# jontio/JAERO

Hardware: NVIDIA H100
Metric: IQ Msamples/s (10.5k OQPSK demod + Viterbi) (higher is better)
Workload: dtype f64

## Files before the change

### jaero_b200/csrc/cfe.cu

```cuda
#include "demod_device.cuh"
#include "fft_device.cuh"
#include <cooperative_groups.h>
#include <cstring>
#include <cstdio>
#include <cstdlib>

namespace jb {

static const int TILE = 16;
static const int MAXN = 128;
static const int CFE_THREADS = 256;

template <bool INV, int R>
__device__ __forceinline__ void stockham_pass(double2 (*s)[MAXN + 1], int n, int Ns, const double2 *__restrict__ tw, int tw_stride)
{
    stockham_pass<INV, R, TILE, MAXN + 1, CFE_THREADS>(s, n, Ns, tw, tw_stride);
}

template <bool INV>
__device__ __forceinline__ void tile_fft(double2 (*s)[MAXN + 1], int n, const double2 *__restrict__ tw, int tw_stride)
{
    stockham_pass<INV, 8>(s, n, 1, tw, tw_stride);
    if (n == 128) { stockham_pass<INV, 4>(s, n, 8, tw, tw_stride); stockham_pass<INV, 4>(s, n, 32, tw, tw_stride); }
    else if (n == 64) stockham_pass<INV, 8>(s, n, 8, tw, tw_stride);
    else stockham_pass<INV, 4>(s, n, 8, tw, tw_stride);
}

template <bool FUSED_INV_SQUARE>
__global__ void __launch_bounds__(CFE_THREADS)
cfe_col_kernel(CfePlan pl, const double2 *__restrict__ src, double2 *__restrict__ dst, size_t src_pitch, int rot, int ring_len, int ch0)
{
    __shared__ double2 s[TILE][MAXN + 1];
    const int ch = blockIdx.y;
    const int c0 = blockIdx.x * TILE;
    const int n1 = pl.n1, n2 = pl.n2, N = pl.nfft;
    const double2 *in = src + (size_t)(ch0 + ch) * src_pitch;
    double2 *out = dst + (size_t)ch * N;
    for (int e = threadIdx.x; e < n1 * TILE; e += CFE_THREADS) {
        const int r = e / TILE, cc = e - r * TILE;
        int n = n2 * r + c0 + cc;
        if (!FUSED_INV_SQUARE) { n += rot; if (n >= ring_len) n -= ring_len; }
        s[cc][r] = in[n];
    }
    __syncthreads();
    if (FUSED_INV_SQUARE) {
        tile_fft<true>(s, n1, pl.tw, N / n1);
        for (int e = threadIdx.x; e < n1 * TILE; e += CFE_THREADS) {
            const int cc = e / n1, r = e - cc * n1;
            const double2 x = s[cc][r];
            s[cc][r] = make_double2(x.x * x.x - x.y * x.y, x.x * x.y + x.y * x.x);
        }
        __syncthreads();
    }
    tile_fft<false>(s, n1, pl.tw, N / n1);
    for (int e = threadIdx.x; e < n1 * TILE; e += CFE_THREADS) {
        const int k1 = e / TILE, cc = e - k1 * TILE;
        const int c = c0 + cc;
        const double2 w = pl.tw[(c * k1) & (N - 1)];
        const double2 x = s[cc][k1];
        out[(size_t)k1 * n2 + c] = make_double2(x.x * w.x - x.y * w.y, x.x * w.y + x.y * w.x);
    }
}

__global__ void __launch_bounds__(CFE_THREADS)
cfe_row_mask_kernel(CfePlan pl, const double2 *__restrict__ src, double2 *__restrict__ dst)
{
    __shared__ double2 s[TILE][MAXN + 1];
    const int ch = blockIdx.y;
    const int r0 = blockIdx.x * TILE;
    const int n1 = pl.n1, n2 = pl.n2, N = pl.nfft;
    const double2 *in = src + (size_t)ch * N;
    double2 *out = dst + (size_t)ch * N;
    for (int e = threadIdx.x; e < n2 * TILE; e += CFE_THREADS) {
        const int rr = e / n2, c = e - rr * n2;
        s[rr][c] = in[(size_t)(r0 + rr) * n2 + c];
    }
    __syncthreads();
    tile_fft<false>(s, n2, pl.tw, N / n2);
    for (int e = threadIdx.x; e < n2 * TILE; e += CFE_THREADS) {
        const int rr = e / n2, k2 = e - rr * n2;
        const int k = (r0 + rr) + n1 * k2;
        double2 x = s[rr][k2];
        if (!pl.is8400) { if (k >= pl.startbin && k <= pl.stopbin) x = make_double2(0.0, 0.0); }
        else { const double w = pl.window[k]; x = make_double2(x.x * w, x.y * w); }
        s[rr][k2] = x;
    }
    __syncthreads();
    tile_fft<true>(s, n2, pl.tw, N / n2);
    for (int e = threadIdx.x; e < n2 * TILE; e += CFE_THREADS) {
        const int rr = e / n2, c = e - rr * n2;
        const int k1 = r0 + rr;
        double2 w = pl.tw[(c * k1) & (N - 1)];
        w.y = -w.y;
        const double2 x = s[rr][c];
        out[(size_t)k1 * n2 + c] = make_double2(x.x * w.x - x.y * w.y, x.x * w.y + x.y * w.x);
    }
}

__global__ void __launch_bounds__(CFE_THREADS)
cfe_row_logmag_kernel(CfePlan pl, DemodParams p, const double2 *__restrict__ src, int ch0)
{
    __shared__ double2 s[TILE][MAXN + 1];
    const int ch = blockIdx.y;
    const int r0 = blockIdx.x * TILE;
    const int n1 = pl.n1, n2 = pl.n2, N = pl.nfft;
    const double2 *in = src + (size_t)ch * N;
    double *y = pl.y + (size_t)(ch0 + ch) * N;
    const bool bigchange = p.I[(size_t)I_ZERO_BB * p.cpad + ch0 + ch] != 0;
    for (int e = threadIdx.x; e < n2 * TILE; e += CFE_THREADS) {
        const int rr = e / n2, c = e - rr * n2;
        s[rr][c] = in[(size_t)(r0 + rr) * n2 + c];
    }
    __syncthreads();
    tile_fft<false>(s, n2, pl.tw, N / n2);
    for (int e = threadIdx.x; e < n2 * TILE; e += CFE_THREADS) {
        const int k2 = e / TILE, rr = e - k2 * TILE;
        const int k1 = r0 + rr;
        const int k2s = (k2 + (n2 >> 1)) & (n2 - 1);
        const int i = k1 + n1 * k2s;
        const double2 x = s[rr][k2];
        const double mag = hypot(x.x, x.y);
        const double yo = bigchange ? 20.0 : y[i];
        y[i] = yo * 0.9 + 0.1 * 10 * log10(fmax(mag, 1.0));
    }
}

__global__ void __launch_bounds__(128)
cfe_search_kernel(CfePlan pl, DemodParams p)
{
    const int lane = threadIdx.x & 31;
    const int ch = blockIdx.x * (blockDim.x >> 5) + (threadIdx.x >> 5);
    if (ch >= p.n_channels) return;
    const double *y = pl.y + (size_t)ch * pl.nfft;
    const int N = pl.nfft, epb = pl.expectedpeakbin;
    double best = 0.0; int besti = 0x7fffffff;
    int i0 = pl.lo;
    if (pl.lo - epb - 1 >= 0 && pl.hi + epb + 1 < N) {
        for (; i0 + 128 <= pl.hi; i0 += 128) {
            double a[4][3], c[4][3];
#pragma unroll
            for (int u = 0; u < 4; u++) {
                const int i = i0 + lane + 32 * u;
#pragma unroll
                for (int j = -1; j <= 1; j++) { a[u][j + 1] = y[i - epb - j]; c[u][j + 1] = y[i + epb + j]; }
            }
#pragma unroll
            for (int u = 0; u < 4; u++) {
                double val = 0;
#pragma unroll
                for (int j = 0; j < 3; j++) val += (a[u][j] + c[u][j]);
                if (val > best) { best = val; besti = i0 + lane + 32 * u; }
            }
        }
    }
    for (int i = i0 + lane; i < pl.hi; i += 32) {
        if ((i < 0) || (i >= N)) continue;
        double val = 0;
        for (int j = -1; j <= 1; j++) {
            if (((i - epb - j) < 0) || ((i + epb + j) >= N)) continue;
            val += (y[i - epb - j] + y[i + epb + j]);
        }
        if (val > best) { best = val; besti = i; }
    }
    for (int off = 16; off > 0; off >>= 1) {
        const double ob = __shfl_xor_sync(0xffffffffu, best, off);
        const int oi = __shfl_xor_sync(0xffffffffu, besti, off);
        if (ob > best || (ob == best && oi < besti)) { best = ob; besti = oi; }
    }
    if (lane == 0) {
        const int zmaxloc = (best > 0.0) ? besti : N / 2;
        const double est = -((double)(zmaxloc - N / 2)) * pl.hzperbin * 0.5;
        p.D[(size_t)D_CFE_EST * p.cpad + ch] = est;
        int &emptying = p.I[(size_t)I_EMPTYING * p.cpad + ch];
        if (emptying <= 0) p.cfe_est_out[ch] = est;
        else { emptying--; p.cfe_est_out[ch] = 0.0; }
        p.I[(size_t)I_ZERO_BB * p.cpad + ch] = 0;
    }
}

namespace cgx = cooperative_groups;

static const int CC_CL = 8, CC_T = 256, CC_SEQ = 16, CC_RS = 143;
static const int CC_BUF = CC_SEQ * CC_RS * 16;
static const int CC_TW2 = 128, CC_TW3 = 152;
static const int CC_SM_TOTAL = 2 * CC_BUF + (128 + 24 + 32) * 16;

__device__ __forceinline__ int cc_ph(int e) { return e + (e >> 3); }

__device__ __forceinline__ double log10_ge1(double x)
{
    const double Lg1 = 6.666666666666735130e-01, Lg2 = 3.999999999940941908e-01, Lg3 = 2.857142874366239149e-01, Lg4 = 2.222219843214978396e-01,
                 Lg5 = 1.818357216161805012e-01, Lg6 = 1.531383769920937332e-01, Lg7 = 1.479819860511658591e-01;
    const double ivln10 = 4.34294481903251816668e-01, log10_2hi = 3.01029995663611771306e-01, log10_2lo = 3.69423907715893078616e-13;
    int hi = __double2hiint(x);
    const int lo = __double2loint(x);
    int k = (hi >> 20) - 1023;
    hi &= 0x000fffff;
    const int i = (hi + 0x95f64) & 0x100000;
    hi |= (i ^ 0x3ff00000);
    k += (i >> 20);
    const double f = __hiloint2double(hi, lo) - 1.0;
    const double s = div_fast(f, 2.0 + f);
    const double z = s * s, w = z * z;
    const double t1 = w * (Lg2 + w * (Lg4 + w * Lg6));
    const double t2 = z * (Lg1 + w * (Lg3 + w * (Lg5 + w * Lg7)));
    const double hfsq = 0.5 * f * f;
    const double lg = f - (hfsq - s * (hfsq + (t2 + t1)));
    const double dk = (double)k;
    return (dk * log10_2lo + ivln10 * lg) + dk * log10_2hi;
}

template <bool INV, bool FIRST, class Store>
__device__ __forceinline__ void cc_fft(double2 *__restrict__ buf, const double2 *__restrict__ tws, Store last)
{
    const int w = threadIdx.x >> 5, l = threadIdx.x & 31;
    if (FIRST) {
        double2 *row = buf + (w + ((l & 16) >> 1)) * CC_RS;
        const int j = l & 15;
        double2 v[8];
#pragma unroll
        for (int t = 0; t < 8; t++) v[t] = row[cc_ph(j + 16 * t)];
        __syncwarp();
        dft8<INV>(v);
#pragma unroll
        for (int t = 0; t < 8; t++) row[cc_ph(8 * j + t)] = v[t];
        __syncwarp();
    }
    double2 *r0 = buf + w * CC_RS, *r1 = buf + (w + 8) * CC_RS;
    auto radix4 = [&](double2 &v0, double2 &v1, double2 &v2, double2 &v3, double2 w1, double2 w2, double2 w3) {
        if (INV) { w1.y = -w1.y; w2.y = -w2.y; w3.y = -w3.y; }
        v1 = c_mul(v1, w1); v2 = c_mul(v2, w2); v3 = c_mul(v3, w3);
        dft4<INV>(v0, v1, v2, v3);
    };
    {
        double2 a0 = r0[cc_ph(l)], a1 = r0[cc_ph(l + 32)], a2 = r0[cc_ph(l + 64)], a3 = r0[cc_ph(l + 96)];
        double2 b0 = r1[cc_ph(l)], b1 = r1[cc_ph(l + 32)], b2 = r1[cc_ph(l + 64)], b3 = r1[cc_ph(l + 96)];
        __syncwarp();
        const int k = l & 7, ob = (l >> 3) * 32 + k;
        const double2 w1 = tws[CC_TW2 + k], w2 = tws[CC_TW2 + 8 + k], w3 = tws[CC_TW2 + 16 + k];
        radix4(a0, a1, a2, a3, w1, w2, w3); radix4(b0, b1, b2, b3, w1, w2, w3);
        r0[cc_ph(ob)] = a0; r0[cc_ph(ob + 8)] = a1; r0[cc_ph(ob + 16)] = a2; r0[cc_ph(ob + 24)] = a3;
        r1[cc_ph(ob)] = b0; r1[cc_ph(ob + 8)] = b1; r1[cc_ph(ob + 16)] = b2; r1[cc_ph(ob + 24)] = b3;
        __syncwarp();
    }
    {
        double2 a0 = r0[cc_ph(l)], a1 = r0[cc_ph(l + 32)], a2 = r0[cc_ph(l + 64)], a3 = r0[cc_ph(l + 96)];
        double2 b0 = r1[cc_ph(l)], b1 = r1[cc_ph(l + 32)], b2 = r1[cc_ph(l + 64)], b3 = r1[cc_ph(l + 96)];
        __syncwarp();
        const double2 w1 = tws[l], w2 = tws[CC_TW3 + l], w3 = tws[3 * l];
        radix4(a0, a1, a2, a3, w1, w2, w3); radix4(b0, b1, b2, b3, w1, w2, w3);
        last(w, l, a0); last(w, l + 32, a1); last(w, l + 64, a2); last(w, l + 96, a3);
        last(w + 8, l, b0); last(w + 8, l + 32, b1); last(w + 8, l + 64, b2); last(w + 8, l + 96, b3);
        __syncwarp();
    }
}

__global__ void __launch_bounds__(CC_T, 2)
cfe_cluster_kernel(CfePlan pl, DemodParams p, int oldest)
{
    extern __shared__ __align__(128) unsigned char cc_smem[];
    double2 *bufA = reinterpret_cast<double2 *>(cc_smem);
    double2 *bufB = reinterpret_cast<double2 *>(cc_smem + CC_BUF);
    double2 *tws = reinterpret_cast<double2 *>(cc_smem + 2 * CC_BUF);
    cgx::cluster_group cluster = cgx::this_cluster();
    const int q = (int)cluster.block_rank();
    const int n_clusters = gridDim.x / CC_CL, cid = blockIdx.x / CC_CL;
    const int N = 16384, ring_len = p.bb_len;
    const double2 *__restrict__ twN = pl.tw;
    if (threadIdx.x < 128) tws[threadIdx.x] = twN[threadIdx.x * (N / 128)];
    else if (threadIdx.x < 128 + 24) { const int e = threadIdx.x - 128, m = e >> 3, k = e & 7; tws[CC_TW2 + e] = twN[(4 * (m + 1) * k) * (N / 128)]; }
    else if (threadIdx.x < 128 + 24 + 32) { const int l = threadIdx.x - 152; tws[CC_TW3 + l] = twN[(2 * l) * (N / 128)]; }
    __syncthreads();
    const double2 *rA[CC_CL], *rB[CC_CL];
#pragma unroll
    for (int s = 0; s < CC_CL; s++) { rA[s] = cluster.map_shared_rank(bufA, s); rB[s] = cluster.map_shared_rank(bufB, s); }
    bool arrived = false;
    cluster.sync();
    for (int ch = cid; ch < p.n_channels; ch += n_clusters) {
        double2 colv[8];
        {
            const double2 *ring = p.bb + (size_t)ch * ring_len;
            const int cc = threadIdx.x & 15, r0i = threadIdx.x >> 4;
#pragma unroll
            for (int i = 0; i < 8; i++) {
                int n = oldest + 128 * (r0i + 16 * i) + 16 * q + cc;
                if (n >= ring_len) n -= ring_len;
                if (n >= ring_len) n -= ring_len;
                colv[i] = ring[n];
            }
        }
        dft8<false>(colv);
        if (arrived) { cluster.barrier_wait(); arrived = false; }
        {
            const int cc = threadIdx.x & 15, r0i = threadIdx.x >> 4;
#pragma unroll
            for (int i = 0; i < 8; i++) bufA[cc * CC_RS + cc_ph(8 * r0i + i)] = colv[i];
        }
        __syncthreads();
        cc_fft<false, false>(bufA, tws, [&](int f, int e, double2 v) { bufA[f * CC_RS + cc_ph(e)] = v; });
        double2 tw8[8];
        {
            const int kk = threadIdx.x & 15, cc = threadIdx.x >> 4;
#pragma unroll
            for (int s = 0; s < 8; s++) tw8[s] = __ldg(&twN[((16 * s + cc) * (16 * q + kk)) & (N - 1)]);
        }
        cluster.sync();
        {
            const int kk = threadIdx.x & 15, cc = threadIdx.x >> 4;
            double2 x[8];
#pragma unroll
            for (int s = 0; s < 8; s++) x[s] = c_mul(rA[s][cc * CC_RS + cc_ph(16 * q + kk)], tw8[s]);
            dft8<false>(x);
#pragma unroll
            for (int s = 0; s < 8; s++) bufB[kk * CC_RS + cc_ph(8 * cc + s)] = x[s];
        }
        __syncthreads();
        cc_fft<false, false>(bufB, tws, [&](int f, int e, double2 v) {
            const int k = (16 * q + f) + 128 * e;
            if (!pl.is8400) { if (k >= pl.startbin && k <= pl.stopbin) v = make_double2(0.0, 0.0); }
            else { const double w = pl.window[k]; v = make_double2(v.x * w, v.y * w); }
            bufB[f * CC_RS + cc_ph(e)] = v;
        });
        cc_fft<true, true>(bufB, tws, [&](int f, int e, double2 v) { bufB[f * CC_RS + cc_ph(e)] = v; });
        {
            const int cc = threadIdx.x & 15, kk = threadIdx.x >> 4;
#pragma unroll
            for (int s = 0; s < 8; s++) tw8[s] = __ldg(&twN[((16 * q + cc) * (16 * s + kk)) & (N - 1)]);
        }
        cluster.sync();
        {
            const int cc = threadIdx.x & 15, kk = threadIdx.x >> 4;
            double2 x[8];
#pragma unroll
            for (int s = 0; s < 8; s++) {
                double2 w = tw8[s]; w.y = -w.y;
                x[s] = c_mul(rB[s][kk * CC_RS + cc_ph(16 * q + cc)], w);
            }
            dft8<true>(x);
#pragma unroll
            for (int s = 0; s < 8; s++) bufA[cc * CC_RS + cc_ph(8 * kk + s)] = x[s];
        }
        __syncthreads();
        cc_fft<true, false>(bufA, tws, [&](int f, int e, double2 v) {
            bufA[f * CC_RS + cc_ph(e)] = make_double2(v.x * v.x - v.y * v.y, v.x * v.y + v.y * v.x);
        });
        cc_fft<false, true>(bufA, tws, [&](int f, int e, double2 v) { bufA[f * CC_RS + cc_ph(e)] = v; });
        {
            const int kk = threadIdx.x & 15, cc = threadIdx.x >> 4;
#pragma unroll
            for (int s = 0; s < 8; s++) tw8[s] = __ldg(&twN[((16 * s + cc) * (16 * q + kk)) & (N - 1)]);
        }
        cluster.sync();
        {
            const int kk = threadIdx.x & 15, cc = threadIdx.x >> 4;
            double2 x[8];
#pragma unroll
            for (int s = 0; s < 8; s++) x[s] = c_mul(rA[s][cc * CC_RS + cc_ph(16 * q + kk)], tw8[s]);
            dft8<false>(x);
#pragma unroll
            for (int s = 0; s < 8; s++) bufB[kk * CC_RS + cc_ph(8 * cc + s)] = x[s];
        }
        cluster.barrier_arrive();
        arrived = true;
        __syncthreads();
        {
            double *y = pl.y + (size_t)ch * N;
            const bool bigchange = p.I[(size_t)I_ZERO_BB * p.cpad + ch] != 0;
            const int kk = threadIdx.x & 15, k2b = threadIdx.x >> 4;
            const int need_lo = pl.lo - pl.expectedpeakbin - 1, need_hi = pl.hi + pl.expectedpeakbin + 1;
            double yo[8];
#pragma unroll
            for (int i = 0; i < 8; i++) {
                const int i_sh = (16 * q + kk) + 128 * ((k2b + 16 * i + 64) & 127);
                yo[i] = (bigchange || i_sh < need_lo || i_sh > need_hi) ? 20.0 : y[i_sh];
            }
            cc_fft<false, false>(bufB, tws, [&](int f, int e, double2 v) { bufB[f * CC_RS + cc_ph(e)] = v; });
            __syncthreads();
#pragma unroll
            for (int i = 0; i < 8; i++) {
                const int k2 = k2b + 16 * i;
                const int i_sh = (16 * q + kk) + 128 * ((k2 + 64) & 127);
                if (i_sh < need_lo || i_sh > need_hi) continue;
                const double2 x = bufB[kk * CC_RS + cc_ph(k2)];
                y[i_sh] = yo[i] * 0.9 + 0.1 * 5 * log10_ge1(fmax(x.x * x.x + x.y * x.y, 1.0));
            }
        }
        __syncthreads();
    }
    if (arrived) cluster.barrier_wait();
    cluster.sync();
}

int cfe_cluster_run(const CfePlan &pl, const DemodParams &p, int oldest, int n_clusters, cudaStream_t s, long long *launches)
{
    cudaLaunchConfig_t cfg;
    memset(&cfg, 0, sizeof cfg);
    cfg.gridDim = dim3((unsigned)(n_clusters * CC_CL)); cfg.blockDim = dim3(CC_T); cfg.dynamicSmemBytes = CC_SM_TOTAL; cfg.stream = s;
    cudaLaunchAttribute at; at.id = cudaLaunchAttributeClusterDimension; at.val.clusterDim.x = CC_CL; at.val.clusterDim.y = 1; at.val.clusterDim.z = 1;
    cfg.attrs = &at; cfg.numAttrs = 1;
    JB_CUDA(cudaLaunchKernelEx(&cfg, cfe_cluster_kernel, pl, p, oldest));
    cfe_search_kernel<<<(p.n_channels + 3) / 4, 128, 0, s>>>(pl, p);
    JB_CUDA(cudaGetLastError());
    *launches += 2;
    return 0;
}
int cfe_cluster_capacity()
{
    if (cudaFuncSetAttribute(cfe_cluster_kernel, cudaFuncAttributeMaxDynamicSharedMemorySize, CC_SM_TOTAL) != cudaSuccess) { cudaGetLastError(); return 0; }
    cudaLaunchConfig_t cfg;
    memset(&cfg, 0, sizeof cfg);
    cfg.gridDim = dim3(CC_CL * 64); cfg.blockDim = dim3(CC_T); cfg.dynamicSmemBytes = CC_SM_TOTAL;
    cudaLaunchAttribute at; at.id = cudaLaunchAttributeClusterDimension; at.val.clusterDim.x = CC_CL; at.val.clusterDim.y = 1; at.val.clusterDim.z = 1;
    cfg.attrs = &at; cfg.numAttrs = 1;
    int n = 0;
    if (cudaOccupancyMaxActiveClusters(&n, cfe_cluster_kernel, &cfg) != cudaSuccess) { cudaGetLastError(); return 0; }
    if (getenv("JAERO_DEBUG")) fprintf(stderr, "[jaero_b200] estimator clusters co-resident: %d x %d CTAs\n", n, CC_CL);
    return n;
}

__global__ void cfe_mark_kernel(int *flag, int value) { __threadfence(); atomicExch(flag, value); }
int cfe_mark_launch(int *flag, int value, cudaStream_t s)
{
    cfe_mark_kernel<<<1, 1, 0, s>>>(flag, value);
    JB_CUDA(cudaGetLastError());
    return 0;
}

int cfe_run(const CfePlan &pl, const DemodParams &p, int oldest, cudaStream_t s, long long *launches)
{
    const int C = p.n_channels;
    for (int ch0 = 0; ch0 < C; ch0 += pl.group) {
        const int g = (C - ch0 < pl.group) ? C - ch0 : pl.group;
        dim3 gc(pl.n2 / TILE, g), gr(pl.n1 / TILE, g);
        cfe_col_kernel<false><<<gc, CFE_THREADS, 0, s>>>(pl, p.bb, pl.work_a, (size_t)p.bb_len, oldest, p.bb_len, ch0);
        cfe_row_mask_kernel<<<gr, CFE_THREADS, 0, s>>>(pl, pl.work_a, pl.work_b);
        cfe_col_kernel<true><<<gc, CFE_THREADS, 0, s>>>(pl, pl.work_b, pl.work_a, (size_t)pl.nfft, 0, pl.nfft, 0);
        cfe_row_logmag_kernel<<<gr, CFE_THREADS, 0, s>>>(pl, p, pl.work_a, ch0);
        *launches += 4;
    }
    cfe_search_kernel<<<(C + 3) / 4, 128, 0, s>>>(pl, p);
    *launches += 1;
    JB_CUDA(cudaGetLastError());
    return 0;
}

}
```

Baseline: 2278.

## Halve CFE cluster block size and fuse 128-point FFT passes in registers

Drops the cluster FFT kernel to 128 threads per block. Each thread now keeps 16 elements of a row in registers and runs the two radix-4 passes, and the radix-8 pass of the next transform, without a shared-memory round trip between them. The window/mask and squaring steps are applied in registers, and remote DSMEM pointers are mapped per access instead of cached in arrays. This trades fewer shared-memory passes and syncs for higher register pressure and half the threads per block, which may reduce occupancy and latency hiding.

Measured after the change: 2427 (median of 6 runs). 1.07x the previous value.

```diff
diff --git a/jaero_b200/csrc/cfe.cu b/jaero_b200/csrc/cfe.cu
--- a/jaero_b200/csrc/cfe.cu
+++ b/jaero_b200/csrc/cfe.cu
@@ -180,7 +180,7 @@
 
 namespace cgx = cooperative_groups;
 
-static const int CC_CL = 8, CC_T = 256, CC_SEQ = 16, CC_RS = 143;
+static const int CC_CL = 8, CC_T = 128, CC_SEQ = 16, CC_RS = 143;
 static const int CC_BUF = CC_SEQ * CC_RS * 16;
 static const int CC_TW2 = 128, CC_TW3 = 152;
 static const int CC_SM_TOTAL = 2 * CC_BUF + (128 + 24 + 32) * 16;
@@ -210,49 +210,57 @@
     return (dk * log10_2lo + ivln10 * lg) + dk * log10_2hi;
 }
 
-template <bool INV, bool FIRST, class Store>
-__device__ __forceinline__ void cc_fft(double2 *__restrict__ buf, const double2 *__restrict__ tws, Store last)
-{
-    const int w = threadIdx.x >> 5, l = threadIdx.x & 31;
-    if (FIRST) {
-        double2 *row = buf + (w + ((l & 16) >> 1)) * CC_RS;
-        const int j = l & 15;
-        double2 v[8];
-#pragma unroll
-        for (int t = 0; t < 8; t++) v[t] = row[cc_ph(j + 16 * t)];
-        __syncwarp();
-        dft8<INV>(v);
-#pragma unroll
-        for (int t = 0; t < 8; t++) row[cc_ph(8 * j + t)] = v[t];
-        __syncwarp();
-    }
-    double2 *r0 = buf + w * CC_RS, *r1 = buf + (w + 8) * CC_RS;
-    auto radix4 = [&](double2 &v0, double2 &v1, double2 &v2, double2 &v3, double2 w1, double2 w2, double2 w3) {
+__device__ __forceinline__ void cc_load16(const double2 *row, int k, double2 (&x)[16])
+{
+#pragma unroll
+    for (int p = 0; p < 16; p++) x[p] = row[cc_ph(k + 8 * p)];
+}
+
+__device__ __forceinline__ void cc_store16(double2 *row, int k, const double2 (&x)[16])
+{
+#pragma unroll
+    for (int p = 0; p < 16; p++) row[cc_ph(k + 8 * p)] = x[p];
+}
+
+template <bool INV>
+__device__ __forceinline__ void cc_pass23(double2 (&x)[16], int k, const double2 *__restrict__ tws)
+{
+    auto radix4 = [](double2 &v0, double2 &v1, double2 &v2, double2 &v3, double2 w1, double2 w2, double2 w3) {
         if (INV) { w1.y = -w1.y; w2.y = -w2.y; w3.y = -w3.y; }
         v1 = c_mul(v1, w1); v2 = c_mul(v2, w2); v3 = c_mul(v3, w3);
         dft4<INV>(v0, v1, v2, v3);
     };
+    double2 y[16];
     {
-        double2 a0 = r0[cc_ph(l)], a1 = r0[cc_ph(l + 32)], a2 = r0[cc_ph(l + 64)], a3 = r0[cc_ph(l + 96)];
-        double2 b0 = r1[cc_ph(l)], b1 = r1[cc_ph(l + 32)], b2 = r1[cc_ph(l + 64)], b3 = r1[cc_ph(l + 96)];
-        __syncwarp();
-        const int k = l & 7, ob = (l >> 3) * 32 + k;
         const double2 w1 = tws[CC_TW2 + k], w2 = tws[CC_TW2 + 8 + k], w3 = tws[CC_TW2 + 16 + k];
-        radix4(a0, a1, a2, a3, w1, w2, w3); radix4(b0, b1, b2, b3, w1, w2, w3);
-        r0[cc_ph(ob)] = a0; r0[cc_ph(ob + 8)] = a1; r0[cc_ph(ob + 16)] = a2; r0[cc_ph(ob + 24)] = a3;
-        r1[cc_ph(ob)] = b0; r1[cc_ph(ob + 8)] = b1; r1[cc_ph(ob + 16)] = b2; r1[cc_ph(ob + 24)] = b3;
-        __syncwarp();
-    }
-    {
-        double2 a0 = r0[cc_ph(l)], a1 = r0[cc_ph(l + 32)], a2 = r0[cc_ph(l + 64)], a3 = r0[cc_ph(l + 96)];
-        double2 b0 = r1[cc_ph(l)], b1 = r1[cc_ph(l + 32)], b2 = r1[cc_ph(l + 64)], b3 = r1[cc_ph(l + 96)];
-        __syncwarp();
-        const double2 w1 = tws[l], w2 = tws[CC_TW3 + l], w3 = tws[3 * l];
-        radix4(a0, a1, a2, a3, w1, w2, w3); radix4(b0, b1, b2, b3, w1, w2, w3);
-        last(w, l, a0); last(w, l + 32, a1); last(w, l + 64, a2); last(w, l + 96, a3);
-        last(w + 8, l, b0); last(w + 8, l + 32, b1); last(w + 8, l + 64, b2); last(w + 8, l + 96, b3);
-        __syncwarp();
-    }
+#pragma unroll
+        for (int m = 0; m < 4; m++) {
+            double2 v0 = x[m], v1 = x[m + 4], v2 = x[m + 8], v3 = x[m + 12];
+            radix4(v0, v1, v2, v3, w1, w2, w3);
+            y[4 * m] = v0; y[4 * m + 1] = v1; y[4 * m + 2] = v2; y[4 * m + 3] = v3;
+        }
+    }
+#pragma unroll
+    for (int u = 0; u < 4; u++) {
+        const int l = k + 8 * u;
+        double2 v0 = y[u], v1 = y[u + 4], v2 = y[u + 8], v3 = y[u + 12];
+        radix4(v0, v1, v2, v3, tws[l], tws[CC_TW3 + l], tws[3 * l]);
+        x[u] = v0; x[u + 4] = v1; x[u + 8] = v2; x[u + 12] = v3;
+    }
+}
+
+template <bool INV>
+__device__ __forceinline__ void cc_pass1_store(const double2 (&x)[16], double2 *row, int k)
+{
+    double2 a[8], b[8];
+#pragma unroll
+    for (int t = 0; t < 8; t++) { a[t] = x[2 * t]; b[t] = x[2 * t + 1]; }
+    dft8<INV>(a);
+    dft8<INV>(b);
+    __syncwarp();
+#pragma unroll
+    for (int t = 0; t < 8; t++) { row[cc_ph(8 * k + t)] = a[t]; row[cc_ph(8 * k + 64 + t)] = b[t]; }
+    __syncwarp();
 }
 
 __global__ void __launch_bounds__(CC_T, 2)
@@ -267,98 +275,137 @@
     const int n_clusters = gridDim.x / CC_CL, cid = blockIdx.x / CC_CL;
     const int N = 16384, ring_len = p.bb_len;
     const double2 *__restrict__ twN = pl.tw;
-    if (threadIdx.x < 128) tws[threadIdx.x] = twN[threadIdx.x * (N / 128)];
-    else if (threadIdx.x < 128 + 24) { const int e = threadIdx.x - 128, m = e >> 3, k = e & 7; tws[CC_TW2 + e] = twN[(4 * (m + 1) * k) * (N / 128)]; }
-    else if (threadIdx.x < 128 + 24 + 32) { const int l = threadIdx.x - 152; tws[CC_TW3 + l] = twN[(2 * l) * (N / 128)]; }
+    for (int t = threadIdx.x; t < 128 + 24 + 32; t += CC_T) {
+        if (t < 128) tws[t] = twN[t * (N / 128)];
+        else if (t < 128 + 24) { const int e = t - 128, m = e >> 3, k = e & 7; tws[CC_TW2 + e] = twN[(4 * (m + 1) * k) * (N / 128)]; }
+        else { const int l = t - 152; tws[CC_TW3 + l] = twN[(2 * l) * (N / 128)]; }
+    }
     __syncthreads();
-    const double2 *rA[CC_CL], *rB[CC_CL];
-#pragma unroll
-    for (int s = 0; s < CC_CL; s++) { rA[s] = cluster.map_shared_rank(bufA, s); rB[s] = cluster.map_shared_rank(bufB, s); }
     bool arrived = false;
     cluster.sync();
+    const int f = threadIdx.x >> 3, k = threadIdx.x & 7;
+    double2 *const rowA = bufA + f * CC_RS, *const rowB = bufB + f * CC_RS;
     for (int ch = cid; ch < p.n_channels; ch += n_clusters) {
-        double2 colv[8];
+        double2 x[16];
+        double2 colv[2][8];
         {
             const double2 *ring = p.bb + (size_t)ch * ring_len;
             const int cc = threadIdx.x & 15, r0i = threadIdx.x >> 4;
 #pragma unroll
-            for (int i = 0; i < 8; i++) {
-                int n = oldest + 128 * (r0i + 16 * i) + 16 * q + cc;
-                if (n >= ring_len) n -= ring_len;
-                if (n >= ring_len) n -= ring_len;
-                colv[i] = ring[n];
-            }
-        }
-        dft8<false>(colv);
+            for (int h = 0; h < 2; h++)
+#pragma unroll
+                for (int i = 0; i < 8; i++) {
+                    int n = oldest + 128 * (r0i + 8 * h + 16 * i) + 16 * q + cc;
+                    if (n >= ring_len) n -= ring_len;
+                    if (n >= ring_len) n -= ring_len;
+                    colv[h][i] = ring[n];
+                }
+        }
+        dft8<false>(colv[0]);
+        dft8<false>(colv[1]);
         if (arrived) { cluster.barrier_wait(); arrived = false; }
         {
             const int cc = threadIdx.x & 15, r0i = threadIdx.x >> 4;
 #pragma unroll
-            for (int i = 0; i < 8; i++) bufA[cc * CC_RS + cc_ph(8 * r0i + i)] = colv[i];
-        }
-        __syncthreads();
-        cc_fft<false, false>(bufA, tws, [&](int f, int e, double2 v) { bufA[f * CC_RS + cc_ph(e)] = v; });
-        double2 tw8[8];
+            for (int h = 0; h < 2; h++)
+#pragma unroll
+                for (int i = 0; i < 8; i++) bufA[cc * CC_RS + cc_ph(8 * (r0i + 8 * h) + i)] = colv[h][i];
+        }
+        __syncthreads();
+        cc_load16(rowA, k, x);
+        cc_pass23<false>(x, k, tws);
+        cc_store16(rowA, k, x);
+        double2 tw8[2][8];
         {
             const int kk = threadIdx.x & 15, cc = threadIdx.x >> 4;
 #pragma unroll
-            for (int s = 0; s < 8; s++) tw8[s] = __ldg(&twN[((16 * s + cc) * (16 * q + kk)) & (N - 1)]);
+            for (int h = 0; h < 2; h++)
+#pragma unroll
+                for (int s = 0; s < 8; s++) tw8[h][s] = __ldg(&twN[((16 * s + cc + 8 * h) * (16 * q + kk)) & (N - 1)]);
         }
         cluster.sync();
         {
+            const int kk = threadIdx.x & 15;
+#pragma unroll
+            for (int h = 0; h < 2; h++) {
+                const int cc = (threadIdx.x >> 4) + 8 * h;
+                double2 v[8];
+#pragma unroll
+                for (int s = 0; s < 8; s++) v[s] = c_mul(cluster.map_shared_rank(bufA, s)[cc * CC_RS + cc_ph(16 * q + kk)], tw8[h][s]);
+                dft8<false>(v);
+#pragma unroll
+                for (int s = 0; s < 8; s++) bufB[kk * CC_RS + cc_ph(8 * cc + s)] = v[s];
+            }
+        }
+        __syncthreads();
+        cc_load16(rowB, k, x);
+        cc_pass23<false>(x, k, tws);
+#pragma unroll
+        for (int e = 0; e < 16; e++) {
+            const int bin = (16 * q + f) + 128 * (k + 8 * e);
+            if (!pl.is8400) { if (bin >= pl.startbin && bin <= pl.stopbin) x[e] = make_double2(0.0, 0.0); }
+            else {
+                const double w = pl.window[bin];
+                x[e] = make_double2(__dmul_rn(x[e].x, w), __dmul_rn(x[e].y, w));
+            }
+        }
+        cc_pass1_store<true>(x, rowB, k);
+        cc_load16(rowB, k, x);
+        cc_pass23<true>(x, k, tws);
+        cc_store16(rowB, k, x);
+        {
+            const int cc = threadIdx.x & 15, kk = threadIdx.x >> 4;
+#pragma unroll
+            for (int h = 0; h < 2; h++)
+#pragma unroll
+                for (int s = 0; s < 8; s++) tw8[h][s] = __ldg(&twN[((16 * q + cc) * (16 * s + kk + 8 * h)) & (N - 1)]);
+        }
+        cluster.sync();
+        {
+            const int cc = threadIdx.x & 15;
+#pragma unroll
+            for (int h = 0; h < 2; h++) {
+                const int kk = (threadIdx.x >> 4) + 8 * h;
+                double2 v[8];
+#pragma unroll
+                for (int s = 0; s < 8; s++) {
+                    double2 w = tw8[h][s]; w.y = -w.y;
+                    v[s] = c_mul(cluster.map_shared_rank(bufB, s)[kk * CC_RS + cc_ph(16 * q + cc)], w);
+                }
+                dft8<true>(v);
+#pragma unroll
+                for (int s = 0; s < 8; s++) bufA[cc * CC_RS + cc_ph(8 * kk + s)] = v[s];
+            }
+        }
+        __syncthreads();
+        cc_load16(rowA, k, x);
+        cc_pass23<true>(x, k, tws);
+#pragma unroll
+        for (int e = 0; e < 16; e++) x[e] = make_double2(x[e].x * x[e].x - x[e].y * x[e].y, x[e].x * x[e].y + x[e].y * x[e].x);
+        cc_pass1_store<false>(x, rowA, k);
+        cc_load16(rowA, k, x);
+        cc_pass23<false>(x, k, tws);
+        cc_store16(rowA, k, x);
+        {
             const int kk = threadIdx.x & 15, cc = threadIdx.x >> 4;
-            double2 x[8];
-#pragma unroll
-            for (int s = 0; s < 8; s++) x[s] = c_mul(rA[s][cc * CC_RS + cc_ph(16 * q + kk)], tw8[s]);
-            dft8<false>(x);
-#pragma unroll
-            for (int s = 0; s < 8; s++) bufB[kk * CC_RS + cc_ph(8 * cc + s)] = x[s];
-        }
-        __syncthreads();
-        cc_fft<false, false>(bufB, tws, [&](int f, int e, double2 v) {
-            const int k = (16 * q + f) + 128 * e;
-            if (!pl.is8400) { if (k >= pl.startbin && k <= pl.stopbin) v = make_double2(0.0, 0.0); }
-            else { const double w = pl.window[k]; v = make_double2(v.x * w, v.y * w); }
-            bufB[f * CC_RS + cc_ph(e)] = v;
-        });
-        cc_fft<true, true>(bufB, tws, [&](int f, int e, double2 v) { bufB[f * CC_RS + cc_ph(e)] = v; });
-        {
-            const int cc = threadIdx.x & 15, kk = threadIdx.x >> 4;
-#pragma unroll
-            for (int s = 0; s < 8; s++) tw8[s] = __ldg(&twN[((16 * q + cc) * (16 * s + kk)) & (N - 1)]);
+#pragma unroll
+            for (int h = 0; h < 2; h++)
+#pragma unroll
+                for (int s = 0; s < 8; s++) tw8[h][s] = __ldg(&twN[((16 * s + cc + 8 * h) * (16 * q + kk)) & (N - 1)]);
         }
         cluster.sync();
         {
-            const int cc = threadIdx.x & 15, kk = threadIdx.x >> 4;
-            double2 x[8];
-#pragma unroll
-            for (int s = 0; s < 8; s++) {
-                double2 w = tw8[s]; w.y = -w.y;
-                x[s] = c_mul(rB[s][kk * CC_RS + cc_ph(16 * q + cc)], w);
-            }
-            dft8<true>(x);
-#pragma unroll
-            for (int s = 0; s < 8; s++) bufA[cc * CC_RS + cc_ph(8 * kk + s)] = x[s];
-        }
-        __syncthreads();
-        cc_fft<true, false>(bufA, tws, [&](int f, int e, double2 v) {
-            bufA[f * CC_RS + cc_ph(e)] = make_double2(v.x * v.x - v.y * v.y, v.x * v.y + v.y * v.x);
-        });
-        cc_fft<false, true>(bufA, tws, [&](int f, int e, double2 v) { bufA[f * CC_RS + cc_ph(e)] = v; });
-        {
-            const int kk = threadIdx.x & 15, cc = threadIdx.x >> 4;
-#pragma unroll
-            for (int s = 0; s < 8; s++) tw8[s] = __ldg(&twN[((16 * s + cc) * (16 * q + kk)) & (N - 1)]);
-        }
-        cluster.sync();
-        {
-            const int kk = threadIdx.x & 15, cc = threadIdx.x >> 4;
-            double2 x[8];
-#pragma unroll
-            for (int s = 0; s < 8; s++) x[s] = c_mul(rA[s][cc * CC_RS + cc_ph(16 * q + kk)], tw8[s]);
-            dft8<false>(x);
-#pragma unroll
-            for (int s = 0; s < 8; s++) bufB[kk * CC_RS + cc_ph(8 * cc + s)] = x[s];
+            const int kk = threadIdx.x & 15;
+#pragma unroll
+            for (int h = 0; h < 2; h++) {
+                const int cc = (threadIdx.x >> 4) + 8 * h;
+                double2 v[8];
+#pragma unroll
+                for (int s = 0; s < 8; s++) v[s] = c_mul(cluster.map_shared_rank(bufA, s)[cc * CC_RS + cc_ph(16 * q + kk)], tw8[h][s]);
+                dft8<false>(v);
+#pragma unroll
+                for (int s = 0; s < 8; s++) bufB[kk * CC_RS + cc_ph(8 * cc + s)] = v[s];
+            }
         }
         cluster.barrier_arrive();
         arrived = true;
@@ -366,23 +413,20 @@
         {
             double *y = pl.y + (size_t)ch * N;
             const bool bigchange = p.I[(size_t)I_ZERO_BB * p.cpad + ch] != 0;
-            const int kk = threadIdx.x & 15, k2b = threadIdx.x >> 4;
             const int need_lo = pl.lo - pl.expectedpeakbin - 1, need_hi = pl.hi + pl.expectedpeakbin + 1;
-            double yo[8];
-#pragma unroll
-            for (int i = 0; i < 8; i++) {
-                const int i_sh = (16 * q + kk) + 128 * ((k2b + 16 * i + 64) & 127);
-                yo[i] = (bigchange || i_sh < need_lo || i_sh > need_hi) ? 20.0 : y[i_sh];
-            }
-            cc_fft<false, false>(bufB, tws, [&](int f, int e, double2 v) { bufB[f * CC_RS + cc_ph(e)] = v; });
-            __syncthreads();
-#pragma unroll
-            for (int i = 0; i < 8; i++) {
-                const int k2 = k2b + 16 * i;
-                const int i_sh = (16 * q + kk) + 128 * ((k2 + 64) & 127);
+            double yo[16];
+#pragma unroll
+            for (int e = 0; e < 16; e++) {
+                const int i_sh = (16 * q + f) + 128 * ((k + 8 * e + 64) & 127);
+                yo[e] = (bigchange || i_sh < need_lo || i_sh > need_hi) ? 20.0 : y[i_sh];
+            }
+            cc_load16(rowB, k, x);
+            cc_pass23<false>(x, k, tws);
+#pragma unroll
+            for (int e = 0; e < 16; e++) {
+                const int i_sh = (16 * q + f) + 128 * ((k + 8 * e + 64) & 127);
                 if (i_sh < need_lo || i_sh > need_hi) continue;
-                const double2 x = bufB[kk * CC_RS + cc_ph(k2)];
-                y[i_sh] = yo[i] * 0.9 + 0.1 * 5 * log10_ge1(fmax(x.x * x.x + x.y * x.y, 1.0));
+                y[i_sh] = yo[e] * 0.9 + 0.1 * 5 * log10_ge1(fmax(x[e].x * x[e].x + x[e].y * x[e].y, 1.0));
             }
         }
         __syncthreads();
```
